# Fil/nd4js

Measured on AMD Instinct MI355X. Metric: fp64 GFLOP/s: matmul N=4096 & SVD N=2048; % of MFMA/HBM peak, higher is better.
Workload: dtype f64; 1 GPU; matmul 4096x4096x4096 fp64, one matrix pair per GPU (BASELINE configs[1]); parallelism=batch-sharded x1, no collective, inputs=uniform(-1,1) seeds 5/6, HBM-resident

## Files before the change

### nd4js_amd/csrc/gemm.hip

```cpp
#include "nd4hip_internal.h"
#include <cstdlib>

typedef double d4 __attribute__((ext_vector_type(4)));
typedef double d2 __attribute__((ext_vector_type(2)));

namespace {

constexpr int BM = 128, BN = 128, BK = 16;
constexpr int LDR = BK + 1;
constexpr int LDK = BN + 16;
constexpr int TILE = BK * LDK;
constexpr int NXCD = 8, GROUP_M = 8;

struct GemmArgs {
  const double* A; const double* B; double* C;
  int M, N, K;
  long lda, ldb, ldc, sA, sB, sC;
  double alpha, beta;
  int tiles_m, tiles_n;
  int lower;
  int kchunk;
  double* Cpart;
};

template <bool VEC, bool FULL>
__device__ __forceinline__ void load_row(d2 (&r)[4], const double* __restrict__ P, long ld,
                                         int x0, int X, int k0, int K, int t) {
  const int kc = k0 + ((t & 7) << 1);
#pragma unroll
  for (int q = 0; q < 4; q++) {
    const int x = x0 + q * 32 + (t >> 3);
    const double* p = P + (long)x * ld + kc;
    if (FULL) {
      r[q] = *reinterpret_cast<const d2*>(p);
    } else if (VEC) {
      d2 v = {0.0, 0.0};
      if (x < X && kc < K) v = *reinterpret_cast<const d2*>(p);
      r[q] = v;
    } else {
      double a = 0.0, b = 0.0;
      if (x < X && kc < K) a = p[0];
      if (x < X && kc + 1 < K) b = p[1];
      r[q].x = a; r[q].y = b;
    }
  }
}
__device__ __forceinline__ void store_row(double* S, const d2 (&r)[4], int t) {
  const int kc = (t & 7) << 1;
#pragma unroll
  for (int q = 0; q < 4; q++) {
    double* s = S + (q * 32 + (t >> 3)) * LDR + kc;
    s[0] = r[q].x; s[1] = r[q].y;
  }
}
template <bool VEC, bool FULL>
__device__ __forceinline__ void load_kmaj(d2 (&r)[4], const double* __restrict__ P, long ld,
                                          int x0, int X, int k0, int K, int t) {
  const int k = k0 + (t >> 4);
#pragma unroll
  for (int q = 0; q < 4; q++) {
    const int x = x0 + q * 32 + ((t & 15) << 1);
    const double* p = P + (long)k * ld + x;
    if (FULL) {
      r[q] = *reinterpret_cast<const d2*>(p);
    } else if (VEC) {
      d2 v = {0.0, 0.0};
      if (k < K && x < X) v = *reinterpret_cast<const d2*>(p);
      r[q] = v;
    } else {
      double a = 0.0, b = 0.0;
      if (k < K && x < X) a = p[0];
      if (k < K && x + 1 < X) b = p[1];
      r[q].x = a; r[q].y = b;
    }
  }
}
__device__ __forceinline__ void store_kmaj(double* S, const d2 (&r)[4], int t) {
#pragma unroll
  for (int q = 0; q < 4; q++)
    *reinterpret_cast<d2*>(S + (t >> 4) * LDK + q * 32 + ((t & 15) << 1)) = r[q];
}

template <bool TA, bool TB, bool VEC, bool FULL>
__global__ __launch_bounds__(256, 2) void dgemm_kernel(GemmArgs g) {
  __shared__ __attribute__((aligned(16))) double lds[4 * TILE];

  const int nwg = g.tiles_m * g.tiles_n;
  int wg;
  {
    const int bid = blockIdx.x, xcd = bid % NXCD, within = bid / NXCD;
    const int q = nwg / NXCD, r = nwg % NXCD;
    wg = (xcd < r ? xcd * (q + 1) : r * (q + 1) + (xcd - r) * q) + within;
  }
  const int per_group = GROUP_M * g.tiles_n;
  const int first_m = (wg / per_group) * GROUP_M;
  const int gsz = min(g.tiles_m - first_m, GROUP_M);
  const int tm = first_m + (wg % per_group) % gsz;
  const int tn = (wg % per_group) / gsz;
  const int m0 = tm * BM, n0 = tn * BN;
  if (g.lower && n0 > m0 + BM - 1) return;

  const long bz = blockIdx.y;
  const double* __restrict__ A = g.A + bz * g.sA;
  const double* __restrict__ B = g.B + bz * g.sB;
  double* __restrict__ C = g.C + bz * g.sC;
  int kbeg = 0, kend = g.K;
  long ldc = g.ldc;
  double alpha = g.alpha, beta = g.beta;
  if (g.kchunk > 0) {
    kbeg = blockIdx.z * g.kchunk; kend = min(g.K, kbeg + g.kchunk);
    C = g.Cpart + ((long)blockIdx.z * gridDim.y + bz) * g.M * g.N;
    ldc = g.N; alpha = 1.0; beta = 0.0;
  }

  const int t = threadIdx.x, lane = t & 63, wave = t >> 6;
  const int wm = (wave >> 1) * 64, wn = (wave & 1) * 64;
  const int fx = lane & 15, fk = lane >> 4;

  d4 acc[4][4];
#pragma unroll
  for (int i = 0; i < 4; i++)
#pragma unroll
    for (int j = 0; j < 4; j++) acc[i][j] = d4{0.0, 0.0, 0.0, 0.0};

  d2 ra[4], rb[4];
  auto gload = [&](int k0) {
    if (TA) load_kmaj<VEC, FULL>(ra, A, g.lda, m0, g.M, k0, kend, t); else load_row<VEC, FULL>(ra, A, g.lda, m0, g.M, k0, kend, t);
    if (TB) load_row<VEC, FULL>(rb, B, g.ldb, n0, g.N, k0, kend, t);  else load_kmaj<VEC, FULL>(rb, B, g.ldb, n0, g.N, k0, kend, t);
  };
  auto sstore = [&](int buf) {
    double* sa = lds + buf * 2 * TILE; double* sb = sa + TILE;
    if (TA) store_kmaj(sa, ra, t); else store_row(sa, ra, t);
    if (TB) store_row(sb, rb, t);  else store_kmaj(sb, rb, t);
  };

  const int nk = (kend - kbeg + BK - 1) / BK;
  gload(kbeg);
  sstore(0);
  __syncthreads();

  for (int kt = 0; kt < nk; kt++) {
    const int cur = kt & 1;
    if (kt + 1 < nk) gload(kbeg + (kt + 1) * BK);
    const double* sa = lds + cur * 2 * TILE;
    const double* sb = sa + TILE;
#pragma unroll
    for (int kk = 0; kk < BK / 4; kk++) {
      double a[4], b[4];
#pragma unroll
      for (int i = 0; i < 4; i++)
        a[i] = TA ? sa[(kk * 4 + fk) * LDK + wm + i * 16 + fx] : sa[(wm + i * 16 + fx) * LDR + kk * 4 + fk];
#pragma unroll
      for (int j = 0; j < 4; j++)
        b[j] = TB ? sb[(wn + j * 16 + fx) * LDR + kk * 4 + fk] : sb[(kk * 4 + fk) * LDK + wn + j * 16 + fx];
      if (kk == BK / 4 - 1 && kt + 1 < nk) {
        sstore(cur ^ 1);
        __builtin_amdgcn_sched_barrier(0);
      }
      __builtin_amdgcn_s_setprio(1);
#pragma unroll
      for (int i = 0; i < 4; i++)
#pragma unroll
        for (int j = 0; j < 4; j++)
          acc[i][j] = __builtin_amdgcn_mfma_f64_16x16x4f64(a[i], b[j], acc[i][j], 0, 0, 0);
      __builtin_amdgcn_s_setprio(0);
    }
    __syncthreads();
  }

#pragma unroll
  for (int i = 0; i < 4; i++)
#pragma unroll
    for (int j = 0; j < 4; j++) {
      const int col = n0 + wn + j * 16 + fx;
#pragma unroll
      for (int r = 0; r < 4; r++) {
        const int row = m0 + wm + i * 16 + fk + 4 * r;
        if (FULL || (row < g.M && col < g.N)) {
          double* c = C + (long)row * ldc + col;
          double v = alpha * acc[i][j][r];
          if (beta != 0.0) v += beta * *c;
          *c = v;
        }
      }
    }
}

constexpr int SK_RT = 1;
constexpr int SK_CT = 2;
constexpr int SK_BM = 4 * 16 * SK_RT, SK_BN = 16 * SK_CT, SK_KSTEPS = 8;

template <bool TB>
__global__ __launch_bounds__(256, 4) void dgemm_smallk_kernel(GemmArgs g) {
  const int tm = blockIdx.x / g.tiles_n, tn = blockIdx.x % g.tiles_n;
  const int m0 = tm * SK_BM, n0 = tn * SK_BN;
  if (g.lower && n0 > m0 + SK_BM - 1) return;
  const int lane = threadIdx.x & 63, w = threadIdx.x >> 6;
  const int fx = lane & 15, fk = lane >> 4;
  const int rbase = m0 + w * 16 * SK_RT;
  if (rbase >= g.M) return;
  const long bz = blockIdx.y;
  const double* __restrict__ A = g.A + bz * g.sA;
  const double* __restrict__ B = g.B + bz * g.sB;
  double* __restrict__ C = g.C + bz * g.sC;
  const int nk = (g.K + 3) >> 2;

  d4 acc[SK_RT][SK_CT];
  const double scale = (g.beta == 0.0) ? 0.0 : g.beta / g.alpha;
#pragma unroll
  for (int i = 0; i < SK_RT; i++)
#pragma unroll
    for (int j = 0; j < SK_CT; j++) {
      const int col = n0 + j * 16 + fx;
#pragma unroll
      for (int r = 0; r < 4; r++) {
        const int row = rbase + i * 16 + fk + 4 * r;
        double c = 0.0;
        if (scale != 0.0 && row < g.M && col < g.N) c = scale * C[(long)row * g.ldc + col];
        acc[i][j][r] = c;
      }
    }
  double a[SK_RT][SK_KSTEPS], b[SK_CT][SK_KSTEPS];
#pragma unroll
  for (int i = 0; i < SK_RT; i++) {
    const int row = rbase + i * 16 + fx;
    const double* ap = A + (long)row * g.lda + fk;
#pragma unroll
    for (int kk = 0; kk < SK_KSTEPS; kk++) a[i][kk] = (row < g.M && kk * 4 + fk < g.K) ? ap[kk * 4] : 0.0;
  }
#pragma unroll
  for (int j = 0; j < SK_CT; j++) {
    const int col = n0 + j * 16 + fx;
#pragma unroll
    for (int kk = 0; kk < SK_KSTEPS; kk++) {
      const int k = kk * 4 + fk;
      double v = 0.0;
      if (col < g.N && k < g.K) v = TB ? B[(long)col * g.ldb + k] : B[(long)k * g.ldb + col];
      b[j][kk] = v;
    }
  }
#pragma unroll
  for (int kk = 0; kk < SK_KSTEPS; kk++)
    if (kk < nk) {
#pragma unroll
      for (int i = 0; i < SK_RT; i++)
#pragma unroll
        for (int j = 0; j < SK_CT; j++) acc[i][j] = __builtin_amdgcn_mfma_f64_16x16x4f64(a[i][kk], b[j][kk], acc[i][j], 0, 0, 0);
    }
  const double alpha = g.alpha;
#pragma unroll
  for (int i = 0; i < SK_RT; i++)
#pragma unroll
    for (int j = 0; j < SK_CT; j++) {
      const int col = n0 + j * 16 + fx;
#pragma unroll
      for (int r = 0; r < 4; r++) {
        const int row = rbase + i * 16 + fk + 4 * r;
        if (row < g.M && col < g.N) C[(long)row * g.ldc + col] = alpha * acc[i][j][r];
      }
    }
}

bool smallk_ok(const GemmArgs& g, bool transA) {
  return !transA && g.K >= 1 && g.K <= 4 * SK_KSTEPS && (g.alpha == 1.0 || g.alpha == -1.0) &&
         (g.beta == 0.0 || g.beta == 1.0 || g.beta == -1.0);
}
template <bool TB>
int launch_smallk(nd4hip_handle* h, GemmArgs g, int64_t batch) {
  g.tiles_m = (g.M + SK_BM - 1) / SK_BM; g.tiles_n = (g.N + SK_BN - 1) / SK_BN;
  ND4_CHECK_ARG((int64_t)g.tiles_m * g.tiles_n < (1ll << 31), "nd4_gemm: too many tiles");
  hipLaunchKernelGGL((dgemm_smallk_kernel<TB>), dim3((unsigned)(g.tiles_m * g.tiles_n), (unsigned)batch, 1), dim3(256, 1, 1), 0, h->stream, g);
  ND4_HIP(hipGetLastError());
  return 0;
}

__global__ __launch_bounds__(256) void dgemm_splitk_reduce(const double* __restrict__ part, int nsplit, long per_split, int M, int N,
                                                            double alpha, double beta, double* __restrict__ Cm, long ldc, long sC) {
  const long b = blockIdx.y;
  const long e = blockIdx.x * 256l + threadIdx.x;
  if (e >= (long)M * N) return;
  double s = 0.0;
  for (int z = 0; z < nsplit; z++) s += part[z * per_split + b * (long)M * N + e];
  double* c = Cm + b * sC + (e / N) * ldc + e % N;
  double v = alpha * s;
  if (beta != 0.0) v += beta * *c;
  *c = v;
}


template <bool TA, bool TB>
int launch(nd4hip_handle* h, const GemmArgs& g, bool vec, int64_t batch) {
  const unsigned nsplit = g.kchunk > 0 ? (unsigned)((g.K + g.kchunk - 1) / g.kchunk) : 1u;
  dim3 grid((unsigned)(g.tiles_m * g.tiles_n), (unsigned)batch, nsplit), block(256, 1, 1);
  const bool full = vec && g.M % BM == 0 && g.N % BN == 0 && g.K % BK == 0 && g.K > 0;
  if (full)     hipLaunchKernelGGL((dgemm_kernel<TA, TB, true, true>), grid, block, 0, h->stream, g);
  else if (vec) hipLaunchKernelGGL((dgemm_kernel<TA, TB, true, false>), grid, block, 0, h->stream, g);
  else          hipLaunchKernelGGL((dgemm_kernel<TA, TB, false, false>), grid, block, 0, h->stream, g);
  ND4_HIP(hipGetLastError());
  return 0;
}

}

int nd4_gemm(nd4hip_handle* h, bool transA, bool transB, int64_t M, int64_t N, int64_t K,
             double alpha, const double* A, int64_t lda, int64_t sA,
             const double* B, int64_t ldb, int64_t sB,
             double beta, double* C, int64_t ldc, int64_t sC, int64_t batch) {
  if (M <= 0 || N <= 0 || batch <= 0) return 0;
  ND4_CHECK_ARG(K >= 0 && M < (1 << 30) && N < (1 << 30) && K < (1 << 30), "nd4_gemm: extent out of range");
  ND4_CHECK_ARG(batch <= 65535, "nd4_gemm: batch %lld exceeds 65535 per launch", (long long)batch);
  GemmArgs g;
  g.A = A; g.B = B; g.C = C; g.M = (int)M; g.N = (int)N; g.K = (int)K;
  g.lda = lda; g.ldb = ldb; g.ldc = ldc; g.sA = sA; g.sB = sB; g.sC = sC;
  g.alpha = alpha; g.beta = beta; g.lower = 0; g.kchunk = 0; g.Cpart = nullptr;
  g.tiles_m = (int)((M + BM - 1) / BM); g.tiles_n = (int)((N + BN - 1) / BN);
  ND4_CHECK_ARG((int64_t)g.tiles_m * g.tiles_n < (1ll << 31), "nd4_gemm: too many tiles");
  if (smallk_ok(g, transA)) return transB ? launch_smallk<true>(h, g, batch) : launch_smallk<false>(h, g, batch);
  Nd4WsScope scope(h);
  const int64_t tiles = (int64_t)g.tiles_m * g.tiles_n * batch;
  int nsplit = 1;
  if (tiles <= 160 && K >= 512) {
    int64_t want = 384 / tiles;
    if (want > K / 256) want = K / 256;
    if (want > 32) want = 32;
    if (want >= 2) {
      int64_t kc = ((K + want - 1) / want + BK - 1) / BK * BK;
      nsplit = (int)((K + kc - 1) / kc);
      void* p = nullptr;
      ND4_TRY(nd4_ws_alloc(h, sizeof(double) * (size_t)nsplit * (size_t)batch * (size_t)M * (size_t)N, &p));
      g.kchunk = (int)kc; g.Cpart = static_cast<double*>(p);
    }
  }
  auto even = [](int64_t v) { return (v & 1) == 0; };
  auto al16 = [](const void* p) { return (reinterpret_cast<uintptr_t>(p) & 15) == 0; };
  const bool vec = al16(A) && al16(B) && even(lda) && even(ldb) && even(sA) && even(sB) &&
                   even(transA ? M : K) && even(transB ? K : N);
  if (transA) ND4_TRY((transB ? launch<true, true>(h, g, vec, batch) : launch<true, false>(h, g, vec, batch)));
  else        ND4_TRY((transB ? launch<false, true>(h, g, vec, batch) : launch<false, false>(h, g, vec, batch)));
  if (g.kchunk > 0) {
    hipLaunchKernelGGL(dgemm_splitk_reduce, dim3((unsigned)((M * N + 255) / 256), (unsigned)batch), dim3(256), 0, h->stream,
                       g.Cpart, nsplit, (long)batch * M * N, (int)M, (int)N, alpha, beta, C, (long)ldc, (long)sC);
    ND4_HIP(hipGetLastError());
  }
  return 0;
}

int nd4_syrk_lower(nd4hip_handle* h, int64_t N, int64_t K, double alpha, const double* A, int64_t lda, int64_t sA,
                   double beta, double* C, int64_t ldc, int64_t sC, int64_t batch) {
  return nd4_gemm_nt_lower(h, N, K, alpha, A, lda, sA, A, lda, sA, beta, C, ldc, sC, batch);
}
int nd4_gemm_nt_lower(nd4hip_handle* h, int64_t N, int64_t K, double alpha, const double* A, int64_t lda, int64_t sA,
                      const double* B, int64_t ldb, int64_t sB, double beta, double* C, int64_t ldc, int64_t sC, int64_t batch) {
  if (N <= 0 || batch <= 0) return 0;
  ND4_CHECK_ARG(K >= 0 && N < (1 << 30) && K < (1 << 30), "nd4_gemm_nt_lower: extent out of range");
  ND4_CHECK_ARG(batch <= 65535, "nd4_gemm_nt_lower: batch %lld exceeds 65535 per launch", (long long)batch);
  GemmArgs g;
  g.A = A; g.B = B; g.C = C; g.M = (int)N; g.N = (int)N; g.K = (int)K;
  g.lda = lda; g.ldb = ldb; g.ldc = ldc; g.sA = sA; g.sB = sB; g.sC = sC;
  g.alpha = alpha; g.beta = beta; g.lower = 1; g.kchunk = 0; g.Cpart = nullptr;
  if (smallk_ok(g, false)) return launch_smallk<true>(h, g, batch);
  g.tiles_m = (int)((N + BM - 1) / BM); g.tiles_n = g.tiles_m;
  auto ok = [](const double* p, int64_t ld, int64_t st) { return (reinterpret_cast<uintptr_t>(p) & 15) == 0 && (ld & 1) == 0 && (st & 1) == 0; };
  const bool vec = ok(A, lda, sA) && ok(B, ldb, sB) && (K & 1) == 0;
  return launch<false, true>(h, g, vec, batch);
}
```

Baseline: 68000 GFLOP/s.

## Software-pipeline LDS fragment reads against MFMA in dgemm main loop

Restructures the dgemm inner loop so LDS fragment reads for the next k-substep are issued before the MFMAs of the current one, using double register fragments and sched_barriers. The global prefetch now runs one tile further ahead, issued right after the barrier. The loop is unrolled by two so buffer indices are compile-time constants. The epilogue is specialized on whether beta is zero and uses precomputed base pointers. This aims to hide LDS latency behind MFMA, at the cost of more registers and removal of the setprio hints.

```diff
diff --git a/nd4js_amd/csrc/gemm.hip b/nd4js_amd/csrc/gemm.hip
--- a/nd4js_amd/csrc/gemm.hip
+++ b/nd4js_amd/csrc/gemm.hip
@@ -81,6 +81,22 @@
     *reinterpret_cast<d2*>(S + (t >> 4) * LDK + q * 32 + ((t & 15) << 1)) = r[q];
 }
 
+template <bool FULL, bool BETA>
+__device__ __forceinline__ void store_c(const d4 (&acc)[4][4], double* __restrict__ c0, long ldc, int rows, int cols, double alpha, double beta) {
+#pragma unroll
+  for (int i = 0; i < 4; i++)
+#pragma unroll
+    for (int j = 0; j < 4; j++)
+#pragma unroll
+      for (int r = 0; r < 4; r++)
+        if (FULL || (i * 16 + 4 * r < rows && j * 16 < cols)) {
+          double* c = c0 + (long)(i * 16 + 4 * r) * ldc + j * 16;
+          double v = alpha * acc[i][j][r];
+          if (BETA) v += beta * *c;
+          *c = v;
+        }
+}
+
 template <bool TA, bool TB, bool VEC, bool FULL>
 __global__ __launch_bounds__(256, 2) void dgemm_kernel(GemmArgs g) {
   __shared__ __attribute__((aligned(16))) double lds[4 * TILE];
@@ -134,56 +150,56 @@
     if (TB) store_row(sb, rb, t);  else store_kmaj(sb, rb, t);
   };
 
+  const double* fa = lds + (TA ? fk * LDK + wm + fx : (wm + fx) * LDR + fk);
+  const double* fb = lds + TILE + (TB ? (wn + fx) * LDR + fk : fk * LDK + wn + fx);
+  auto fread = [&](double (&a)[4], double (&b)[4], int buf, int kk) __attribute__((always_inline)) {
+#pragma unroll
+    for (int i = 0; i < 4; i++) a[i] = fa[buf * 2 * TILE + (TA ? kk * 4 * LDK + i * 16 : i * 16 * LDR + kk * 4)];
+#pragma unroll
+    for (int j = 0; j < 4; j++) b[j] = fb[buf * 2 * TILE + (TB ? j * 16 * LDR + kk * 4 : kk * 4 * LDK + j * 16)];
+    __builtin_amdgcn_sched_barrier(0);
+  };
+  auto mma = [&](const double (&a)[4], const double (&b)[4]) __attribute__((always_inline)) {
+#pragma unroll
+    for (int i = 0; i < 4; i++)
+#pragma unroll
+      for (int j = 0; j < 4; j++)
+        acc[i][j] = __builtin_amdgcn_mfma_f64_16x16x4f64(a[i], b[j], acc[i][j], 0, 0, 0);
+    __builtin_amdgcn_sched_barrier(0);
+  };
+
   const int nk = (kend - kbeg + BK - 1) / BK;
   gload(kbeg);
   sstore(0);
+  if (nk > 1) gload(kbeg + BK);
   __syncthreads();
 
-  for (int kt = 0; kt < nk; kt++) {
-    const int cur = kt & 1;
-    if (kt + 1 < nk) gload(kbeg + (kt + 1) * BK);
-    const double* sa = lds + cur * 2 * TILE;
-    const double* sb = sa + TILE;
-#pragma unroll
-    for (int kk = 0; kk < BK / 4; kk++) {
-      double a[4], b[4];
-#pragma unroll
-      for (int i = 0; i < 4; i++)
-        a[i] = TA ? sa[(kk * 4 + fk) * LDK + wm + i * 16 + fx] : sa[(wm + i * 16 + fx) * LDR + kk * 4 + fk];
-#pragma unroll
-      for (int j = 0; j < 4; j++)
-        b[j] = TB ? sb[(wn + j * 16 + fx) * LDR + kk * 4 + fk] : sb[(kk * 4 + fk) * LDK + wn + j * 16 + fx];
-      if (kk == BK / 4 - 1 && kt + 1 < nk) {
-        sstore(cur ^ 1);
-        __builtin_amdgcn_sched_barrier(0);
-      }
-      __builtin_amdgcn_s_setprio(1);
-#pragma unroll
-      for (int i = 0; i < 4; i++)
-#pragma unroll
-        for (int j = 0; j < 4; j++)
-          acc[i][j] = __builtin_amdgcn_mfma_f64_16x16x4f64(a[i], b[j], acc[i][j], 0, 0, 0);
-      __builtin_amdgcn_s_setprio(0);
-    }
-    __syncthreads();
-  }
-
-#pragma unroll
-  for (int i = 0; i < 4; i++)
-#pragma unroll
-    for (int j = 0; j < 4; j++) {
-      const int col = n0 + wn + j * 16 + fx;
-#pragma unroll
-      for (int r = 0; r < 4; r++) {
-        const int row = m0 + wm + i * 16 + fk + 4 * r;
-        if (FULL || (row < g.M && col < g.N)) {
-          double* c = C + (long)row * ldc + col;
-          double v = alpha * acc[i][j][r];
-          if (beta != 0.0) v += beta * *c;
-          *c = v;
-        }
-      }
-    }
+  double a0[4], b0[4], a1[4], b1[4];
+  fread(a0, b0, 0, 0);
+  auto kstep = [&](int cur, int kt, bool more, bool more2) __attribute__((always_inline)) {
+    fread(a1, b1, cur, 1); mma(a0, b0);
+    fread(a0, b0, cur, 2); mma(a1, b1);
+    fread(a1, b1, cur, 3);
+    if (more) { sstore(cur ^ 1); __builtin_amdgcn_sched_barrier(0); }
+    mma(a0, b0);
+    if (more) {
+      __syncthreads();
+      if (more2) gload(kbeg + (kt + 2) * BK);
+      fread(a0, b0, cur ^ 1, 0);
+    }
+    mma(a1, b1);
+  };
+  int kt = 0;
+  for (; kt + 2 < nk; kt += 2) {
+    kstep(0, kt, true, true);
+    kstep(1, kt + 1, true, kt + 3 < nk);
+  }
+  if (kt < nk) kstep(0, kt, kt + 1 < nk, false);
+  if (kt + 1 < nk) kstep(1, kt + 1, false, false);
+
+  double* c0 = C + (long)(m0 + wm + fk) * ldc + n0 + wn + fx;
+  if (beta != 0.0) store_c<FULL, true>(acc, c0, ldc, g.M - (m0 + wm + fk), g.N - (n0 + wn + fx), alpha, beta);
+  else             store_c<FULL, false>(acc, c0, ldc, g.M - (m0 + wm + fk), g.N - (n0 + wn + fx), alpha, beta);
 }
 
 constexpr int SK_RT = 1;
```

New measurement: 70830 GFLOP/s (median of 6 runs). 4.2% higher.
